# tanderson92/Fast_solver_Lippmann_Schwinger

Measured on NVIDIA B200. Metric: ls_operator_applies_per_s_2d, higher is better.
Workload: dtype f64

## Files before the change

fast_solver_lippmann_schwinger_b200/csrc/line_kernels.cuh:

```cuda
#pragma once
#include "fft_engine.cuh"
#include <cooperative_groups.h>

namespace lsk {
using namespace lsfft;

template <int N> struct GeoA {
    static constexpr int E = Cfg<N>::E;
    static constexpr int T = N / E;
    static constexpr int LPC = (T >= 128) ? 1 : 128 / T;
    static constexpr int THREADS = T * LPC;
};
template <int N> struct GeoB {
    static constexpr int E = Cfg<N>::E;
    static constexpr int T = N / E;
    static constexpr int LB = LinesB<N>::value;
    static constexpr int GPC = (LB * T >= 128) ? 1 : 128 / (LB * T);
    static constexpr int LPC = LB * GPC;
    static constexpr int THREADS = LB * T * GPC;
};
#ifndef LS_INV512_MINB
#define LS_INV512_MINB 2
#endif
template <int N, bool MODE_B> struct MinB {
    static constexpr int TH = MODE_B ? GeoB<N>::THREADS : GeoA<N>::THREADS;
    static constexpr int value = (TH <= 128) ? 3 : ((MODE_B && GeoB<N>::LB == 4 && TH == 256) ? 2 : 1);
};
template <int N, bool MODE_B> struct MinBInv {
    static constexpr int value = (N == 512 && MinB<N, MODE_B>::value == 3) ? LS_INV512_MINB : MinB<N, MODE_B>::value;
};

template <int N, bool MODE_B> struct Map;
template <int N> struct Map<N, false> {
    typedef GeoA<N> G;
    typedef LayA<N> Lay;
    int line, t;
    Lay lay;
    __device__ __forceinline__ Map() {
        line = threadIdx.x / G::T;
        t = threadIdx.x % G::T;
        lay.base = line * N;
    }
    __device__ __forceinline__ int lay_lam() const { return 0; }
};
template <int N> struct Map<N, true> {
    typedef GeoB<N> G;
    typedef LayB<N> Lay;
    int line, t;
    Lay lay;
    __device__ __forceinline__ Map() {
        constexpr int LB = G::LB;
        int grp = threadIdx.x / (LB * G::T);
        int w = threadIdx.x % (LB * G::T);
        lay.lam = w % LB;
        t = w / LB;
// ... 161 lines not shown
            cd gv[E];
            fft_fwd<N>(v, t, r, ex, mp.lay, tw, [&]() {
                const cd* g = MODE_B ? gsrc + ((long)(mp.line / LBK) * nr + rr) * UNIT + mp.lay_lam()
                                     : gsrc + ((long)mp.line * nr + rr) * UNIT;
                constexpr int gs = LBK;
#pragma unroll
                for (int e = 0; e < E; ++e) gv[e] = __ldg(&g[(t + T * e) * gs]);
            });
#pragma unroll
            for (int e = 0; e < E; ++e) v[e] = cmul(v[e], gv[e]);
        } else {
        fft_fwd<N>(v, t, r, ex, mp.lay, tw);
        mbar_wait(bar, (unsigned)(rr & 1));
        if (MODE_B) {
            const cd* g = gb + sm_group_off(mp);
#pragma unroll
            for (int e = 0; e < E; ++e) v[e] = cmul(v[e], g[(t + T * e) * LBK + mp.lay_lam()]);
        } else {
            const cd* g = gb + goff;
#pragma unroll
            for (int e = 0; e < E; ++e) v[e] = cmul(v[e], g[t + T * e]);
        }
        }
        fft_inv<N>(v, t, r, ex, mp.lay, tw, [&]() {
            if (GSM && rr + 1 < nr && threadIdx.x == 0) {
                fence_proxy_async();
                issue_g(rr + 1);
            }
        });
        if (ASM == 0) {
            demod_accumulate<N>(acc, v, r);
        } else if (r == 0) {
#pragma unroll
            for (int a = 0; a < AR; ++a) acc[a] = v[a];
#pragma unroll
            for (int a = AR; a < E; ++a) accs[(a - AR) * TH] = v[a];
        } else {
            acc[0] = cadd(acc[0], v[0]);
#pragma unroll
            for (int a = 1; a < AR; ++a) acc[a] = cfmac(v[a], c64(r * a * (16 / E)), acc[a]);
#pragma unroll
            for (int a = AR; a < E; ++a) accs[(a - AR) * TH] = cfmac(v[a], c64(r * a * (16 / E)), accs[(a - AR) * TH]);
        }
    }
    cd* o = out + line_out(la, L) + (long)t * la.out_es;
#pragma unroll
    for (int a = 0; a < AR; ++a) o[(long)(a * T) * la.out_es] = acc[a];
#pragma unroll
    for (int a = AR; a < E; ++a) o[(long)(a * T) * la.out_es] = accs[(a - AR) * TH];
}

template <int N, int MINB, int GL>
__global__ void __launch_bounds__(GeoA<N>::THREADS, MINB)
k_mid_swap(const cd* in, cd* out, const cd* __restrict__ G, const cd* __restrict__ TAB, const LineAddr la, long line0) {
    typedef Map<N, false> M;
    constexpr int E = Cfg<N>::E, T = N / E, LPC = M::G::LPC, TH = GeoA<N>::THREADS;
    extern __shared__ __align__(128) cd sm[];
    M mp;
    cd* ex = sm;
    cd* hold = sm + LPC * N + threadIdx.x;
    cd* tw1 = sm + 2 * LPC * N;
    load_tw1<N>(tw1, TAB);
    const long L = line0 + (long)blockIdx.x * LPC + mp.line;
    const int t = mp.t;
    const TwState<N> tw = make_tw<N>(t, TAB, tw1);
    const cd* gline = G + L * 2L * N;
    cd v[E];
    {
        const cd* p = in + line_in(la, L) + (long)t * la.in_es;
#pragma unroll
        for (int a = 0; a < E; ++a) v[a] = p[(long)(a * T) * la.in_es];
#pragma unroll
        for (int a = 0; a < E; ++a) hold[a * TH] = v[a];
    }
    __syncthreads();
#pragma unroll 1
    for (int rr = 0; rr < 2; ++rr) {
        const int r = 2 * rr;
        const cd* g = gline + (long)rr * N;
        if constexpr (GL == 0) {
            cd gv[E];
            fft_fwd<N>(v, t, r, ex, mp.lay, tw, [&]() {
#pragma unroll
                for (int e = 0; e < E; ++e) gv[e] = __ldg(&g[t + T * e]);
            });
#pragma unroll
            for (int e = 0; e < E; ++e) v[e] = cmul(v[e], gv[e]);
        } else {
            fft_fwd<N>(v, t, r, ex, mp.lay, tw, [&]() {
                if ((t & 7) == 0) {
#pragma unroll
                    for (int e = 0; e < E; ++e) prefetch_l2(&g[t + T * e]);
                }
            });
#pragma unroll
            for (int e = 0; e < E; ++e) v[e] = cmul(v[e], __ldg(&g[t + T * e]));
        }
        fft_inv<N>(v, t, r, ex, mp.lay, tw);
        if (rr == 0) {
#pragma unroll
            for (int a = 0; a < E; ++a) {
                const cd xa = hold[a * TH];
                hold[a * TH] = v[a];
                v[a] = xa;
            }
        }
    }
    cd* o = out + line_out(la, L) + (long)t * la.out_es;
    o[0] = cadd(hold[0], v[0]);
#pragma unroll
    for (int a = 1; a < E; ++a) o[(long)(a * T) * la.out_es] = cfmac(v[a], c64(2 * a * (16 / E)), hold[a * TH]);
}

__device__ __forceinline__ void cp_async16(void* dst_smem, const void* src) {
    asm volatile("cp.async.cg.shared.global [%0], [%1], 16;" ::"r"(smem_u32(dst_smem)), "l"(src) : "memory");
}
__device__ __forceinline__ void cp_async_commit() { asm volatile("cp.async.commit_group;" ::: "memory"); }
template <int K> __device__ __forceinline__ void cp_async_wait() { asm volatile("cp.async.wait_group %0;" ::"n"(K) : "memory"); }

template <int N, bool MODE_B, int PF = 0>
__global__ void __launch_bounds__(MODE_B ? GeoB<N>::THREADS : GeoA<N>::THREADS, MinBInv<N, MODE_B>::value)
k_inv_pruned(const cd* __restrict__ in, const cd* bsrc, cd* out, const cd* __restrict__ TAB, double scale,
             const LineAddr la, long line0) {
    typedef Map<N, MODE_B> M;
    constexpr int E = Cfg<N>::E, T = N / E, LPC = M::G::LPC;
    extern __shared__ __align__(128) cd sm[];
    M mp;
    cd* ex = sm + sm_group_off(mp);
    cd* tw1 = sm + LPC * N;
    load_tw1<N>(tw1, TAB);
    const long L = line0 + (long)blockIdx.x * LPC + mp.line;
    const int t = mp.t;
    const TwState<N> tw = make_tw<N>(t, TAB, tw1);
    __syncthreads();
    const long in_base = line_in(la, L), out_base = line_out(la, L);
    cd acc[E];
    const int nr = la.nr, rstep = 4 / la.nr;
    constexpr int TH = MODE_B ? GeoB<N>::THREADS : GeoA<N>::THREADS;
    cd* stg = sm + LPC * N + EngTab<N>::TW1N + threadIdx.x;
#pragma unroll 1
    for (int rr = 0; rr < nr; ++rr) {
        const int r = rr * rstep;
        cd v[E];
        const cd* p = in + in_base;
        if (PF == 2 && rr > 0) {
            cp_async_wait<0>();
#pragma unroll
            for (int e = 0; e < E; ++e) v[e] = stg[TH * e];
        } else {
#pragma unroll
            for (int e = 0; e < E; ++e) v[e] = p[slot_off(la, (long)(rr * N + t + T * e), la.in_es)];
        }
        if (PF == 2) {
            if (rr + 1 < nr) {
#pragma unroll
                for (int e = 0; e < E; ++e) cp_async16(&stg[TH * e], &p[slot_off(la, (long)((rr + 1) * N + t + T * e), la.in_es)]);
                cp_async_commit();
            } else if (bsrc != nullptr) {
#pragma unroll
                for (int a = 0; a < E; ++a) cp_async16(&stg[TH * a], &bsrc[out_base + (long)(a * T + t) * la.out_es]);
                cp_async_commit();
            }
        } else if (!PF) {
        } else if (rr + 1 < nr) {
// ... 12 lines not shown
    }
#pragma unroll
    for (int a = 0; a < E; ++a) {
        long off = out_base + (long)(a * T + t) * la.out_es;
        cd res = cscale(acc[a], scale);
        if (bsrc != nullptr) {
            if (PF == 2 && a == 0) cp_async_wait<0>();
            const cd bv = (PF == 2) ? stg[TH * a] : bsrc[off];
            res = make_double2(__fma_rn(acc[a].x, scale, bv.x), __fma_rn(acc[a].y, scale, bv.y));
        }
        out[off] = res;
    }
}

}

namespace lsk {

template <class K> inline cudaError_t smem_optin(K kernel, int smem, unsigned long long& done) {
    int dev = 0;
    cudaError_t e = cudaGetDevice(&dev);
    if (e != cudaSuccess) return e;
    const unsigned long long bit = 1ull << (dev & 63);
    if (done & bit) return cudaSuccess;
    e = cudaFuncSetAttribute(kernel, cudaFuncAttributeMaxDynamicSharedMemorySize, smem);
    if (e == cudaSuccess) done |= bit;
    return e;
}

template <int N, bool B>
inline cudaError_t launch_fwd(cudaStream_t s, long nlines, const cd* in, const double* nu, cd* out, const cd* TAB,
                              const LineAddr& la) {
    constexpr int smem = Smem<N, B>::fwd_bytes;
    constexpr int LPC = Smem<N, B>::LPC, TH = B ? GeoB<N>::THREADS : GeoA<N>::THREADS;
    static unsigned long long optin = 0;
    { cudaError_t e = smem_optin(k_fwd_pruned<N, B>, smem, optin); if (e != cudaSuccess) return e; }
    k_fwd_pruned<N, B><<<(unsigned)(nlines / LPC), TH, smem, s>>>(in, nu, out, TAB, la, 0);
    return cudaPeekAtLastError();
}

template <int N, bool B, bool GSM>
inline cudaError_t launch_mid(cudaStream_t s, long nlines, const cd* in, cd* out, const cd* G, const cd* TAB,
                              const LineAddr& la) {
    constexpr int smem = GSM ? Smem<N, B>::mid_bytes : Smem<N, B>::mid_bytes_direct;
    constexpr int LPC = Smem<N, B>::LPC, TH = B ? GeoB<N>::THREADS : GeoA<N>::THREADS;
    static unsigned long long optin = 0;
    constexpr int MB = (B && GeoB<N>::LB == 4) ? 2 : 1;
    { cudaError_t e = smem_optin(k_mid_fused<N, B, GSM, MB>, smem, optin); if (e != cudaSuccess) return e; }
    k_mid_fused<N, B, GSM, MB><<<(unsigned)(nlines / LPC), TH, smem, s>>>(in, out, G, TAB, la, 0);
    return cudaPeekAtLastError();
}

template <int N, int MINB, int GL>
inline cudaError_t launch_mid_swap(cudaStream_t s, long nlines, const cd* in, cd* out, const cd* G, const cd* TAB,
                                   const LineAddr& la) {
    constexpr int smem = (2 * GeoA<N>::LPC * N + EngTab<N>::TW1N) * (int)sizeof(cd);
    static unsigned long long optin = 0;
    { cudaError_t e = smem_optin(k_mid_swap<N, MINB, GL>, smem, optin); if (e != cudaSuccess) return e; }
    k_mid_swap<N, MINB, GL><<<(unsigned)(nlines / GeoA<N>::LPC), GeoA<N>::THREADS, smem, s>>>(in, out, G, TAB, la, 0);
    return cudaPeekAtLastError();
}

template <int N, bool B, int PF = 0>
inline cudaError_t launch_inv(cudaStream_t s, long nlines, const cd* in, const cd* bsrc, cd* out, const cd* TAB,
                              double scale, const LineAddr& la) {
    constexpr int smem = Smem<N, B>::fwd_bytes + (PF == 2 ? Smem<N, B>::LPC * N * (int)sizeof(cd) : 0);
    constexpr int LPC = Smem<N, B>::LPC, TH = B ? GeoB<N>::THREADS : GeoA<N>::THREADS;
    static unsigned long long optin = 0;
    { cudaError_t e = smem_optin(k_inv_pruned<N, B, PF>, smem, optin); if (e != cudaSuccess) return e; }
    k_inv_pruned<N, B, PF><<<(unsigned)(nlines / LPC), TH, smem, s>>>(in, bsrc, out, TAB, scale, la, 0);
    return cudaPeekAtLastError();
}

}
```

fast_solver_lippmann_schwinger_b200/csrc/op2d.cu:

```cuda
#include "ls_common.cuh"
#include "op2d_base.cuh"
#include "line_kernels.cuh"
#include "gv_spectrum2d.cuh"
#ifdef LS_EXPERIMENTS
#include "line_kernels_experiments.cuh"
#endif

using namespace ls;
using namespace lsk;

namespace {

struct Op2D : Op2DBase {
    int nr = 4;
    long pn = 0, pm = 0;
    double* d_nu = nullptr;
    cd* d_G = nullptr;
    cd* d_TABn = nullptr; cd* d_TABm = nullptr;
    cd* d_A = nullptr;
    cd* d_C = nullptr;
    int cw = 1;
    int apply_dev(const cd* b, cd* y, int mode) override;
};

__global__ void k_scale(cd* a, long n, double s) {
    for (long i = (long)blockIdx.x * blockDim.x + threadIdx.x; i < n; i += (long)gridDim.x * blockDim.x) {
        cd v = a[i];
        a[i] = make_double2(v.x * s, v.y * s);
    }
}

__global__ void k_permute_g2d(const cd* __restrict__ gin, cd* __restrict__ gout,
                              const int* __restrict__ fx, const int* __restrict__ fy,
                              long n, long m, long ne, long me, double scale) {
    long idx = (long)blockIdx.x * blockDim.x + threadIdx.x;
    long total = ne * me;
    if (idx >= total) return;
    long sy = idx % m;
    long ry = (idx / m) % 4;
    long sx = idx / (4 * m);
    long kx = 4L * fx[sx % n] + sx / n;
    long ky = 4L * fy[sy] + ry;
    long ix = (kx + ne / 2) % ne, iy = (ky + me / 2) % me;
    cd v = gin[ix + ne * iy];
    gout[idx] = make_double2(v.x * scale, v.y * scale);
}

__global__ void k_fill_g2d(cd* __restrict__ gout, const int* __restrict__ fx, const int* __restrict__ fy,
                           long n, long m, long ne, long me, double scale, Gv2dParams p) {
    long idx = (long)blockIdx.x * blockDim.x + threadIdx.x;
    long total = ne * me;
    if (idx >= total) return;
    long sy = idx % m;
    long ry = (idx / m) % 4;
    long sx = idx / (4 * m);
    long kx = 4L * fx[sx % n] + sx / n;
    long ky = 4L * fy[sy] + ry;
    long ix = (kx + ne / 2) % ne, iy = (ky + me / 2) % me;
    cd v = gtrunc2d_eval(p, ix, iy, ne, me);
    gout[idx] = make_double2(v.x * scale, v.y * scale);
}
__global__ void k_fill_g2d_centred(cd* __restrict__ gout, long ne, long me, Gv2dParams p) {
    long idx = (long)blockIdx.x * blockDim.x + threadIdx.x;
    if (idx >= ne * me) return;
    gout[idx] = gtrunc2d_eval(p, idx % ne, idx / ne, ne, me);
}

template <int N> int launch_fwd(Op2D* op, const cd* b, const double* nu) {
    constexpr int smem = Smem<N, false>::fwd_bytes;
    static unsigned long long optin = 0;
    LS_CUDA_TRY(smem_optin(k_fwd_pruned<N, false>, smem, optin));
    dim3 grid((unsigned)(op->m / GeoA<N>::LPC));
    LineAddr la{1L << 40, op->n, 0, 1, op->pn, 0, 1};
    la.nr = op->nr;
    op->phase_begin(0);
    k_fwd_pruned<N, false><<<grid, GeoA<N>::THREADS, smem, op->stream>>>(b, nu, op->d_A, op->d_TABn, la, 0);
    op->phase_end();
    op->launches++;
    return LS_OK;
}
template <int N, bool GSM, int MINB, int ASM = 0> int launch_mid_v(Op2D* op) {
    static int extra = -1;
    if (extra < 0) { const char* e = getenv("LS_P2_EXTRA_SMEM"); extra = e ? atoi(e) : 0; }
    const int smem = (GSM ? Smem<N, false>::mid_bytes : Smem<N, false>::mid_bytes_direct) + extra
                     + ASM * GeoA<N>::THREADS * (int)sizeof(cd);
    static unsigned long long optin = 0;
    LS_CUDA_TRY(smem_optin(k_mid_fused<N, false, GSM, MINB, ASM>, smem, optin));
    dim3 grid((unsigned)(op->pn / GeoA<N>::LPC));
    const long cw = op->cw;
    LineAddr la{cw, 1, cw, op->pn, 1, cw * op->m, cw};
    la.nr = op->nr;
    op->phase_begin(1);
    k_mid_fused<N, false, GSM, MINB, ASM><<<grid, GeoA<N>::THREADS, smem, op->stream>>>(
        op->d_A, op->d_C, op->d_G, op->d_TABm, la, 0);
    op->phase_end();
    op->launches++;
    return LS_OK;
}
#ifdef LS_EXPERIMENTS
template <int N, int ASM> int launch_mid_dual(Op2D* op) {
    const int smem = (3 * GeoA<N>::LPC * N + EngTab<N>::TW1N + ASM * GeoA<N>::THREADS) * (int)sizeof(cd);
    static unsigned long long optin = 0;
    LS_CUDA_TRY(smem_optin(k_mid_fused_dual<N, ASM>, smem, optin));
    dim3 grid((unsigned)(op->ne / GeoA<N>::LPC));
    op->phase_begin(1);
    k_mid_fused_dual<N, ASM><<<grid, GeoA<N>::THREADS, smem, op->stream>>>(
        op->d_A, op->d_C, op->d_G, op->d_TABm, LineAddr{1L << 40, 1, 0, op->ne, op->m, 0, 1}, 0);
    op->phase_end();
    op->launches++;
    return LS_OK;
}
#endif
template <int N> int launch_mid_swap_op(Op2D* op) {
    const long cw = op->cw;
    LineAddr la{cw, 1, cw, op->pn, 1, cw * op->m, cw};
    la.nr = 2;
    static int gl = -1, minb = -1;
    if (gl < 0) { const char* e = getenv("LS_P2_GLOAD"); gl = e ? atoi(e) : 0; }
    if (minb < 0) { const char* e = getenv("LS_P2_MINB"); minb = e ? atoi(e) : 0; }
    const int use_minb = minb ? minb : (N <= 256 ? 3 : 2);
    constexpr int MB = (GeoA<N>::THREADS <= 128 ? 3 : 1);
    op->phase_begin(1);
    cudaError_t e;
    constexpr int MB2 = (MB == 3 ? 2 : 1);
    if (use_minb == 2 || MB == 1) e = gl ? lsk::launch_mid_swap<N, MB2, 1>(op->stream, op->pn, op->d_A, op->d_C, op->d_G, op->d_TABm, la)
                                     : lsk::launch_mid_swap<N, MB2, 0>(op->stream, op->pn, op->d_A, op->d_C, op->d_G, op->d_TABm, la);
    else e = gl ? lsk::launch_mid_swap<N, MB, 1>(op->stream, op->pn, op->d_A, op->d_C, op->d_G, op->d_TABm, la)
                : lsk::launch_mid_swap<N, MB, 0>(op->stream, op->pn, op->d_A, op->d_C, op->d_G, op->d_TABm, la);
    op->phase_end();
    op->launches++;
    LS_CUDA_TRY(e);
    return LS_OK;
}
template <int N> int launch_mid(Op2D* op) {
    static int kernel = -1;
    if (kernel < 0) { const char* e = getenv("LS_P2_KERNEL"); kernel = e ? atoi(e) : 1; }
    if (op->nr == 2 && kernel == 1) return launch_mid_swap_op<N>(op);
#ifndef LS_EXPERIMENTS
    return launch_mid_v<N, false, 1>(op);
#else
    static int variant = -1;
    if (op->nr != 4) return launch_mid_v<N, false, 1>(op);
    if (variant < 0) { const char* e = getenv("LS_P2_VARIANT"); variant = e ? atoi(e) : 1; }
    if (variant == 0) return launch_mid_v<N, true, 1>(op);
    if constexpr (N == 2048) if (variant == 8) {
        static int ctas = -1;
        if (ctas < 0) { const char* e = getenv("LS_P2_CTAS"); ctas = e ? atoi(e) : 2 * 148; }
        op->phase_begin(1);
        cudaError_t e = launch_mid_persist<N>(op->stream, op->ne, op->d_A, op->d_C, op->d_G, op->d_TABm,
                                              LineAddr{1L << 40, 1, 0, op->ne, op->m, 0, 1}, ctas);
        op->phase_end();
        op->launches++;
        LS_CUDA_TRY(e);
        return LS_OK;
    }
    if constexpr (N == 2048) if (variant == 6 || variant == 7) {
        op->phase_begin(1);
        const LineAddr la{1L << 40, 1, 0, op->ne, op->m, 0, 1};
        cudaError_t e = (variant == 6) ? launch_mid_cluster<N, false, 3>(op->stream, op->ne, op->d_A, op->d_C, op->d_G, op->d_TABm, la)
                                       : launch_mid_cluster<N, false, 4>(op->stream, op->ne, op->d_A, op->d_C, op->d_G, op->d_TABm, la);
        op->phase_end();
        op->launches++;
        LS_CUDA_TRY(e);
        return LS_OK;
    }
    if constexpr (N == 2048) { if (variant == 5) return launch_mid_dual<N, 4>(op); }
    if (variant == 2) return launch_mid_v<N, false, 3, 4>(op);
    if (variant == 3) return launch_mid_v<N, false, 3, 2>(op);
    return launch_mid_v<N, false, 1>(op);
#endif
}
template <int N, int PF> int launch_inv_v(Op2D* op, const cd* bsrc, cd* y, double scale) {
    constexpr int smem = Smem<N, false>::fwd_bytes + (PF == 2 ? Smem<N, false>::LPC * N * (int)sizeof(cd) : 0);
    static unsigned long long optin = 0;
    LS_CUDA_TRY(smem_optin(k_inv_pruned<N, false, PF>, smem, optin));
    dim3 grid((unsigned)(op->m / GeoA<N>::LPC));
    const long cw = op->cw;
    int cshift = 0;
    while ((1L << cshift) < cw) ++cshift;
    LineAddr la{1L << 40, cw, 0, 1, op->n, 0, 1};
    la.split_shift = cshift; la.split_stride = cw * op->m;
    la.nr = op->nr;
    op->phase_begin(2);
    k_inv_pruned<N, false, PF><<<grid, GeoA<N>::THREADS, smem, op->stream>>>(op->d_C, bsrc, y, op->d_TABn, scale, la, 0);
    op->phase_end();
    op->launches++;
    return LS_OK;
}
template <int N> int launch_inv(Op2D* op, const cd* bsrc, cd* y, double scale) {
    static int stage = -1;
// ... 50 lines not shown
    }

int compact_spectrum(Op2D* op, cd* g4s) {
    const long n = op->n, m = op->m;
    cudaStream_t s = op->stream;
    cudaError_t e = cudaSuccess;
    cd *t1 = nullptr, *g2 = nullptr, *t2 = nullptr, *G2 = nullptr;
    int rc;
    if ((rc = op->dmalloc((void**)&t1, (size_t)(4 * n) * (2 * m) * sizeof(cd)))) return rc;
    for (int c = 0; c <= 3; c += 3) {
        LineAddr la{1L << 40, 4 * m, 0, 1, 2 * m, 0, 1};
        la.nr = 4; la.cblock = c;
        cd* outp = t1 + (c ? m : 0);
#define S1(N) launch_inv<N, false>(s, 4 * n, g4s, nullptr, outp, op->d_TABm, 1.0, la)
        LS_DISPATCH_E(m, S1);
        LS_CUDA_TRY(e);
    }
    LS_CUDA_TRY(cudaStreamSynchronize(s));
    op->dfree(g4s);
    if ((rc = op->dmalloc((void**)&g2, (size_t)(2 * n) * (2 * m) * sizeof(cd)))) return rc;
    for (int c = 0; c <= 3; c += 3) {
        LineAddr la{1L << 40, 1, 0, 2 * m, 2 * n, 0, 1};
        la.nr = 4; la.cblock = c;
        cd* outp = g2 + (c ? n : 0);
#define S2(N) launch_inv<N, false>(s, 2 * m, t1, nullptr, outp, op->d_TABn, 1.0, la)
        LS_DISPATCH_E(n, S2);
        LS_CUDA_TRY(e);
    }
    LS_CUDA_TRY(cudaStreamSynchronize(s));
    op->dfree(t1);
    if ((rc = op->dmalloc((void**)&t2, (size_t)(2 * n) * (2 * m) * sizeof(cd)))) return rc;
    if ((rc = op->dmalloc((void**)&G2, (size_t)(2 * n) * (2 * m) * sizeof(cd)))) return rc;
    {
        LineAddr la{1L << 40, 2 * n, 0, 1, 2 * n, 0, 1};
        la.nr = 2; la.full2 = 1;
#define S3(N) launch_fwd<N, false>(s, 2 * m, g2, nullptr, t2, op->d_TABn, la)
        LS_DISPATCH_E(n, S3);
        LS_CUDA_TRY(e);
    }
    {
        LineAddr la{1L << 40, 1, 0, 2 * n, 2 * m, 0, 1};
        la.nr = 2; la.full2 = 1;
#define S4(N) launch_fwd<N, false>(s, 2 * n, t2, nullptr, G2, op->d_TABm, la)
        LS_DISPATCH_E(m, S4);
        LS_CUDA_TRY(e);
    }
    k_scale<<<148 * 8, 256, 0, s>>>(G2, (2 * n) * (2 * m), 1.0 / ((double)(2 * n) * (double)(2 * m)));
    LS_CUDA_TRY(cudaStreamSynchronize(s));
    op->dfree(g2);
    op->dfree(t2);
    op->d_G = G2;
    op->nr = 2;
    return LS_OK;
}

}

extern "C" {

static int op2d_create_impl(ls_handle* out, int64_t n, int64_t m, int64_t ne, int64_t me,
                            const double* nu, const ls_cdouble* gfft, double omega, int quadrule, int flags,
                            double L, double Lp);

int ls_op2d_create(ls_handle* out, int64_t n, int64_t m, int64_t ne, int64_t me,
                   const double* nu, const ls_cdouble* gfft, double omega, int quadrule, int flags) {
    LS_REQUIRE(out && nu && gfft, LS_ERR_INVALID, "ls_op2d_create: null pointer");
    return op2d_create_impl(out, n, m, ne, me, nu, gfft, omega, quadrule, flags, 0.0, 0.0);
}

int ls_op2d_create_gv(ls_handle* out, int64_t n, int64_t m, const double* nu, double omega, double L, double Lp, int flags) {
    LS_REQUIRE(out && nu, LS_ERR_INVALID, "ls_op2d_create_gv: null pointer");
    LS_REQUIRE(L > 0 && Lp > 0 && omega > 0, LS_ERR_INVALID, "ls_op2d_create_gv: L, Lp and k must be positive");
    return op2d_create_impl(out, n, m, 4 * n, 4 * m, nu, nullptr, omega, LS_QUAD_GREENGARD_VICO, flags, L, Lp);
}

static int op2d_create_impl(ls_handle* out, int64_t n, int64_t m, int64_t ne, int64_t me,
                            const double* nu, const ls_cdouble* gfft, double omega, int quadrule, int flags,
                            double L, double Lp) {
    LS_REQUIRE(n > 0 && m > 0 && ne > 0 && me > 0, LS_ERR_INVALID, "ls_op2d_create: non-positive size");
    LS_REQUIRE(quadrule == LS_QUAD_TRAPEZOIDAL || quadrule == LS_QUAD_GREENGARD_VICO, LS_ERR_INVALID,
               "ls_op2d_create: unknown quadRule %d", quadrule);
    if (quadrule == LS_QUAD_TRAPEZOIDAL) {
        LS_REQUIRE(ne == 2 * n - 1 && me == 2 * m - 1, LS_ERR_INVALID,
                   "ls_op2d_create: trapezoidal needs ne = 2n-1, me = 2m-1 (FastConvolution.jl:183)");
        return create_op2d_generic(out, n, m, ne, me, nu, gfft, omega, quadrule);
    }
    LS_REQUIRE(ne == 4 * n && me == 4 * m, LS_ERR_INVALID,
               "ls_op2d_create: Greengard_Vico needs ne = 4n, me = 4m (FastConvolution.jl:201)");
    if (!(fft_size_supported(n) && fft_size_supported(m)) || (flags & LS_FLAG_FORCE_GENERIC)) {
        if (gfft) return create_op2d_generic(out, n, m, ne, me, nu, gfft, omega, quadrule);
        LS_REQUIRE(ne + n - 1 <= 4096 && me + m - 1 <= 4096, LS_ERR_UNSUPPORTED,
                   "ls_op2d_create_gv: n=%ld, m=%ld: the general-size GPU path serves 5n - 1 <= 4096", (long)n, (long)m);
        cd* d_g = nullptr;
        LS_CUDA_TRY(cudaMalloc((void**)&d_g, (size_t)ne * me * sizeof(cd)));
        const Gv2dParams gp = gv2d_params(L, Lp, omega);
        k_fill_g2d_centred<<<(unsigned)(((size_t)ne * me + 255) / 256), 256>>>(d_g, ne, me, gp);
        cudaError_t ge = cudaDeviceSynchronize();
        int grc = ge == cudaSuccess ? create_op2d_generic(out, n, m, ne, me, nu, nullptr, omega, quadrule, d_g) : LS_ERR_CUDA;
        if (ge != cudaSuccess) set_error("spectrum generation failed: %s", cudaGetErrorString(ge));
        cudaFree(d_g);
        return grc;
    }

    Op2D* op = new Op2D();
    int rc = op->init_base(KIND_OP2D);
    if (rc) { delete op; return rc; }
    op->n = n; op->m = m; op->ne = ne; op->me = me; op->omega = omega; op->quadrule = quadrule;
    const size_t N = (size_t)n * m, NE = (size_t)ne * me;
#define TRY(x) do { rc = (x); if (rc) { delete op; return rc; } } while (0)
    TRY(op->dupload((void**)&op->d_nu, nu, N * sizeof(double)));
    {
        auto Tn = engine_table((int)n), Tm = engine_table((int)m);
        TRY(op->dupload((void**)&op->d_TABn, Tn.data(), Tn.size() * sizeof(cd)));
        TRY(op->dupload((void**)&op->d_TABm, Tm.data(), Tm.size() * sizeof(cd)));
    }
    {
        auto fx = slot_freq((int)n), fy = slot_freq((int)m);
        int *d_fx = nullptr, *d_fy = nullptr;
        cd* d_gin = nullptr;
        TRY(op->dupload((void**)&d_fx, fx.data(), fx.size() * sizeof(int)));
        TRY(op->dupload((void**)&d_fy, fy.data(), fy.size() * sizeof(int)));
        TRY(op->dmalloc((void**)&op->d_G, NE * sizeof(cd)));
        const int th = 256;
        if (gfft) {
            TRY(op->dupload((void**)&d_gin, gfft, NE * sizeof(cd)));
            k_permute_g2d<<<(unsigned)((NE + th - 1) / th), th, 0, op->stream>>>(
                d_gin, op->d_G, d_fx, d_fy, n, m, ne, me, 1.0 / ((double)ne * (double)me));
        } else {
            k_fill_g2d<<<(unsigned)((NE + th - 1) / th), th, 0, op->stream>>>(
                op->d_G, d_fx, d_fy, n, m, ne, me, 1.0 / ((double)ne * (double)me), gv2d_params(L, Lp, omega));
        }
        cudaError_t e = cudaStreamSynchronize(op->stream);
        if (e != cudaSuccess) { set_error("spectrum set-up failed: %s", cudaGetErrorString(e)); delete op; return LS_ERR_CUDA; }
        if (d_gin) op->dfree(d_gin);
        op->dfree(d_fx); op->dfree(d_fy);
    }
    op->nr = 4;
    if (!(flags & LS_FLAG_PAD4)) {
        cd* g4s = op->d_G;
        op->d_G = nullptr;
        TRY(compact_spectrum(op, g4s));
    }
    op->pn = op->nr * n; op->pm = op->nr * m;
    {
        const char* ev = getenv("LS_C_INTERLEAVE");
        int cw = ev ? atoi(ev) : 4;
        if (cw != 1 && cw != 2 && cw != 4 && cw != 8) cw = 4;
        const char* pv = getenv("LS_P2_VARIANT");
        if (op->nr == 4 && pv && atoi(pv) >= 5) cw = 1;
        op->cw = cw;
    }
    TRY(op->dmalloc((void**)&op->d_A, (size_t)op->pn * m * sizeof(cd)));
    TRY(op->dmalloc((void**)&op->d_C, (size_t)op->pn * m * sizeof(cd)));
    TRY(op->dmalloc((void**)&op->d_b, N * sizeof(cd)));
    TRY(op->dmalloc((void**)&op->d_y, N * sizeof(cd)));
#undef TRY
    *out = reinterpret_cast<ls_handle>(op);
    return LS_OK;
}

int ls_op2d_apply(ls_handle h, const ls_cdouble* b, ls_cdouble* y, int mode, int memloc) {
    LS_REQUIRE(h && b && y, LS_ERR_INVALID, "ls_op2d_apply: null argument");
    Op2DBase* op = reinterpret_cast<Op2DBase*>(h);
    LS_REQUIRE(op->kind == KIND_OP2D, LS_ERR_INVALID, "ls_op2d_apply: not a 2-D operator handle");
    LS_REQUIRE(mode == LS_APPLY_FASTCONVOLUTION || mode == LS_APPLY_FFTCONVOLUTION, LS_ERR_INVALID,
               "ls_op2d_apply: unknown mode %d", mode);
    if (mode == LS_APPLY_FFTCONVOLUTION)
        LS_REQUIRE(op->n == op->m, LS_ERR_INVALID,
                   "FFTconvolution pads (ne,ne) and crops (n,n): square grids only (FastConvolution.jl:139-151)");
    LS_CUDA_TRY(cudaSetDevice(op->device));
    const size_t bytes = (size_t)op->n * op->m * sizeof(cd);
    if (memloc == LS_MEM_DEVICE) {
        return op->apply_dev(reinterpret_cast<const cd*>(b), reinterpret_cast<cd*>(y), mode);
    }
    LS_REQUIRE(memloc == LS_MEM_HOST, LS_ERR_INVALID, "ls_op2d_apply: unknown memloc %d", memloc);
    LS_CUDA_TRY(cudaMemcpyAsync(op->d_b, b, bytes, cudaMemcpyHostToDevice, op->stream));
    int rc = op->apply_dev(op->d_b, op->d_y, mode);
    if (rc) return rc;
    LS_CUDA_TRY(cudaMemcpyAsync(y, op->d_y, bytes, cudaMemcpyDeviceToHost, op->stream));
    LS_CUDA_TRY(cudaStreamSynchronize(op->stream));
    return LS_OK;
}

}
```

fast_solver_lippmann_schwinger_b200/_lib.py:

```python
from __future__ import annotations

import ctypes as C
import os
import re

import numpy as np

HERE = os.path.dirname(os.path.abspath(__file__))
LIB_PATH = os.environ.get("LS_CUDA_LIB") or os.path.join(HERE, "lib", "libls_cuda.so")
HEADER_PATH = os.path.join(os.path.dirname(HERE), "include", "ls_cuda.h")

LS_OK = 0
LS_ERR_INVALID, LS_ERR_UNSUPPORTED, LS_ERR_CUDA, LS_ERR_NOMEM, LS_ERR_NCCL, LS_ERR_CALLBACK = -1, -2, -3, -4, -5, -6
MEM_HOST, MEM_DEVICE = 0, 1
QUAD_TRAPEZOIDAL, QUAD_GREENGARD_VICO = 0, 1
APPLY_FASTCONVOLUTION, APPLY_FFTCONVOLUTION = 0, 1

QUADRULES = {"trapezoidal": QUAD_TRAPEZOIDAL, "Greengard_Vico": QUAD_GREENGARD_VICO}


class CDouble(C.Structure):
    _fields_ = [("re", C.c_double), ("im", C.c_double)]

    @classmethod
# ... 37 lines not shown
    vp, i64, dbl, ci = C.c_void_p, C.c_int64, C.c_double, C.c_int
    sig = {
        "ls_version": (ci, []),
        "ls_last_error": (C.c_char_p, []),
        "ls_device_count": (ci, [C.POINTER(ci)]),
        "ls_set_device": (ci, [ci]),
        "ls_dev_alloc": (ci, [C.POINTER(vp), C.c_size_t]),
        "ls_dev_free": (ci, [vp]),
        "ls_memcpy_h2d": (ci, [vp, vp, C.c_size_t]),
        "ls_memcpy_d2h": (ci, [vp, vp, C.c_size_t]),
        "ls_host_alloc_pinned": (ci, [C.POINTER(vp), C.c_size_t]),
        "ls_host_free_pinned": (ci, [vp]),
        "ls_op2d_create": (ci, [C.POINTER(vp), i64, i64, i64, i64, vp, vp, dbl, ci, ci]),
        "ls_op2d_create_gv": (ci, [C.POINTER(vp), i64, i64, vp, dbl, dbl, dbl, ci]),
        "ls_op2d_apply": (ci, [vp, vp, vp, ci, ci]),
        "ls_op3d_create": (ci, [C.POINTER(vp), i64, i64, i64, i64, i64, i64, vp, vp, dbl, dbl, dbl, ci]),
        "ls_op3d_apply": (ci, [vp, vp, vp, ci, ci]),
        "ls_op3d_info": (ci, [vp, C.POINTER(ci), C.POINTER(ci), C.POINTER(ci)]),
        "ls_nccl_unique_id": (ci, [vp]),
        "ls_op3d_create_dist": (ci, [C.POINTER(vp), i64, i64, i64, vp, dbl, dbl, dbl, ci, ci, vp, ci]),
        "ls_op_size": (ci, [vp, C.POINTER(i64)]),
        "ls_spm_create": (ci, [C.POINTER(vp), i64, i64, vp, vp, vp]),
        "ls_spm_create_dist": (ci, [C.POINTER(vp), vp, i64, i64, vp, vp, vp]),
        "ls_spm_mv": (ci, [vp, CDouble, vp, CDouble, vp, ci]),
        "ls_spm_info": (ci, [vp, C.POINTER(i64), C.POINTER(i64), C.POINTER(i64), C.POINTER(ci), C.POINTER(ci)]),
        "ls_krylov_create": (ci, [C.POINTER(vp), i64]),
        "ls_krylov_set_orth": (ci, [vp, ci]),
        "ls_zdotc": (ci, [vp, vp, vp, C.POINTER(CDouble)]),
        "ls_dznrm2": (ci, [vp, vp, C.POINTER(dbl)]),
        "ls_zaxpy": (ci, [vp, CDouble, vp, vp]),
        "ls_zscal": (ci, [vp, CDouble, vp]),
        "ls_mgs_step": (ci, [vp, vp, i64, ci, vp, vp]),
        "ls_gmres": (ci, [vp, vp, vp, SOLVE_CB, vp, vp, vp, ci, i64, dbl, dbl, ci, vp, i64,
                          C.POINTER(i64), C.POINTER(ci), C.POINTER(i64), ci]),
        "ls_msp_factor": (ci, [C.POINTER(vp), i64, i64, vp, vp, vp]),
        "ls_msp_factor3d": (ci, [C.POINTER(vp), i64, i64, i64, vp, vp, vp]),
        "ls_msp_solve": (ci, [vp, vp, vp, ci]),
        "ls_msp_info": (ci, [vp, C.POINTER(i64), C.POINTER(ci), C.POINTER(dbl)]),
        "ls_msp_plan": (ci, [vp, C.c_char_p, i64]),
        "ls_gmres_msp": (ci, [vp, vp, vp, vp, vp, vp, ci, i64, dbl, dbl, ci, vp, i64,
                              C.POINTER(i64), C.POINTER(ci), C.POINTER(i64), ci]),
        "ls_krylov_last_precond_host_seconds": (ci, [vp, C.POINTER(dbl)]),
        "ls_sample_rows": (ci, [vp, vp, vp, ci, vp, i64]),
        "ls_gram": (ci, [vp, vp, i64, ci, vp]),
        "ls_gather_rows": (ci, [vp, vp, i64, ci, vp, ci, vp]),
        "ls_destroy": (ci, [vp]),
        "ls_sync": (ci, [vp]),
        "ls_timer_start": (ci, [vp]),
        "ls_timer_stop": (ci, [vp, C.POINTER(C.c_float)]),
        "ls_launch_count": (ci, [vp, C.POINTER(i64)]),
        "ls_profile_enable": (ci, [vp, ci]),
        "ls_profile_read": (ci, [vp, C.POINTER(dbl), C.POINTER(i64), ci]),
        "ls_test_fft_lines": (ci, [i64, i64, vp, vp, ci]),
        "ls_test_device_peaks": (ci, [C.POINTER(dbl), C.POINTER(dbl), C.POINTER(dbl)]),
    }
    for name, (res, args) in sig.items():
        fn = getattr(L, name)
        fn.restype = res
        fn.argtypes = args
    L._signatures = sig
    _lib = L
    return L


def check(rc):
    if rc == LS_OK:
        return
    msg = lib().ls_last_error().decode("utf-8", "replace")
    if rc == LS_ERR_UNSUPPORTED:
        raise LSUnsupported(rc, msg)
    raise LSCudaError(rc, msg)


def ptr(a):
    if a is None:
        return None
    if isinstance(a, np.ndarray):
        return a.ctypes.data_as(C.c_void_p)
    if isinstance(a, DeviceBuffer):
        return C.c_void_p(a.ptr)
    return C.c_void_p(int(a))


class DeviceBuffer:

    def __init__(self, nbytes):
        p = C.c_void_p()
        check(lib().ls_dev_alloc(C.byref(p), nbytes))
        self.ptr = p.value
        self.nbytes = nbytes

    @classmethod
    def from_host(cls, arr):
        arr = np.ascontiguousarray(arr)
        buf = cls(arr.nbytes)
        check(lib().ls_memcpy_h2d(C.c_void_p(buf.ptr), ptr(arr), arr.nbytes))
        return buf

    def to_host(self, dtype=np.complex128, count=None):
        dtype = np.dtype(dtype)
        count = self.nbytes // dtype.itemsize if count is None else count
        out = np.empty(count, dtype=dtype)
        check(lib().ls_memcpy_d2h(ptr(out), C.c_void_p(self.ptr), count * dtype.itemsize))
        return out

    def offset(self, nbytes):
# ... 37 lines not shown
```

include/ls_cuda.h:

```cpp
#ifndef LS_CUDA_H
#define LS_CUDA_H

#include <stddef.h>
#include <stdint.h>

#ifdef __cplusplus
extern "C" {
#endif

typedef struct { double re, im; } ls_cdouble;
typedef struct ls_handle_s* ls_handle;

#define LS_OK               0
#define LS_ERR_INVALID     -1
#define LS_ERR_UNSUPPORTED -2
#define LS_ERR_CUDA        -3
#define LS_ERR_NOMEM       -4
#define LS_ERR_NCCL        -5
#define LS_ERR_CALLBACK    -6

#define LS_FLAG_FORCE_GENERIC 1
#define LS_FLAG_PAD4          2

#define LS_MEM_HOST   0
// ... 35 lines not shown
int ls_op3d_apply(ls_handle h, const ls_cdouble* b, ls_cdouble* y, int mode, int memloc);

int ls_spm_create(ls_handle* out, int64_t nrows, int64_t ncols, const int64_t* colptr,
                  const int64_t* rowval, const ls_cdouble* nzval);
int ls_spm_create_dist(ls_handle* out, ls_handle op, int64_t nrows_local, int64_t halo, const int64_t* colptr,
                       const int64_t* rowval, const ls_cdouble* nzval);
int ls_spm_mv(ls_handle A, ls_cdouble alpha, const ls_cdouble* x, ls_cdouble beta, ls_cdouble* y, int memloc);
int ls_spm_info(ls_handle A, int64_t* nrows, int64_t* ncols, int64_t* nnz, int* format, int* nclasses);

int ls_krylov_create(ls_handle* out, int64_t n);
int ls_krylov_set_orth(ls_handle k, int orth_meth);
int ls_zdotc(ls_handle k, const ls_cdouble* x, const ls_cdouble* y, ls_cdouble* result);
int ls_dznrm2(ls_handle k, const ls_cdouble* x, double* result);
int ls_zaxpy(ls_handle k, ls_cdouble alpha, const ls_cdouble* x, ls_cdouble* y);
int ls_zscal(ls_handle k, ls_cdouble alpha, ls_cdouble* x);
int ls_mgs_step(ls_handle k, const ls_cdouble* V, int64_t ldv, int kcols, ls_cdouble* w, ls_cdouble* hcol);

typedef int (*ls_solve_cb)(void* user, ls_cdouble* v_inout, int64_t n);

int ls_gmres(ls_handle krylov, ls_handle op, ls_handle As, ls_solve_cb msp_solve, void* user,
             const ls_cdouble* b, ls_cdouble* x, int restart, int64_t maxiter, double reltol,
             double abstol, int initially_zero, double* resnorm_hist, int64_t hist_cap,
             int64_t* niter, int* converged, int64_t* mv_products, int memloc);

int ls_msp_factor(ls_handle* out, int64_t n, int64_t m, const int64_t* colptr, const int64_t* rowval,
                  const ls_cdouble* nzval);
int ls_msp_factor3d(ls_handle* out, int64_t n, int64_t m, int64_t l, const int64_t* colptr, const int64_t* rowval,
                    const ls_cdouble* nzval);
int ls_msp_solve(ls_handle msp, const ls_cdouble* rhs, ls_cdouble* x, int memloc);
int ls_msp_info(ls_handle msp, int64_t* factor_bytes, int* depth, double* factor_seconds);
int ls_msp_plan(ls_handle msp, char* buf, int64_t cap);
int ls_gmres_msp(ls_handle krylov, ls_handle op, ls_handle As, ls_handle msp,
                 const ls_cdouble* b, ls_cdouble* x, int restart, int64_t maxiter, double reltol,
                 double abstol, int initially_zero, double* resnorm_hist, int64_t hist_cap,
                 int64_t* niter, int* converged, int64_t* mv_products, int memloc);
int ls_krylov_last_precond_host_seconds(ls_handle krylov, double* seconds);

int ls_sample_rows(ls_handle krylov, ls_handle op, const int64_t* indS, int s, ls_cdouble* V_dev, int64_t ldv);
int ls_gram(ls_handle krylov, const ls_cdouble* V_dev, int64_t ldv, int s, ls_cdouble* gram_host);
int ls_gather_rows(ls_handle krylov, const ls_cdouble* V_dev, int64_t ldv, int s, const int64_t* idx, int nidx, ls_cdouble* out_host);

int ls_destroy(ls_handle h);
int ls_sync(ls_handle h);
int ls_timer_start(ls_handle h);
int ls_timer_stop(ls_handle h, float* elapsed_ms);
int ls_launch_count(ls_handle h, int64_t* count);

int ls_profile_enable(ls_handle h, int on);
int ls_profile_read(ls_handle h, double* ms_per_phase, int64_t* launches_per_phase, int nphase);

int ls_test_fft_lines(int64_t N, int64_t nlines, const ls_cdouble* in_host, ls_cdouble* out_host,
                      int inverse_roundtrip);

int ls_test_device_peaks(double* dfma_tflops, double* dadd_tinst, double* copy_gbs);

#ifdef __cplusplus
}
#endif
#endif
```

Before: 2846.

## Add TMA-tiled mid-phase kernel loading transposed line tiles via tensor maps

Adds a new middle-stage kernel that uses TMA bulk tensor loads to pull a tile of strided lines into swizzled shared memory. It then runs the forward FFT, spectrum multiply and inverse FFT in place and writes the tile back with TMA 3D stores into the interleaved C layout. The goal is to replace scattered strided global accesses with coalesced bulk copies and cut address-generation overhead. It becomes the default for sizes 1024–2048 when tensor maps encode successfully. In exchange it adds shared memory for the tile and serialises the load, compute and store phases within each CTA.

Result: faster. 2960 (median of 6 runs) (+4.0%).

```diff
diff --git a/fast_solver_lippmann_schwinger_b200/csrc/line_kernels.cuh b/fast_solver_lippmann_schwinger_b200/csrc/line_kernels.cuh
--- a/fast_solver_lippmann_schwinger_b200/csrc/line_kernels.cuh
+++ b/fast_solver_lippmann_schwinger_b200/csrc/line_kernels.cuh
@@ -1,6 +1,7 @@
 #pragma once
 #include "fft_engine.cuh"
 #include <cooperative_groups.h>
+#include <cuda.h>
 
 namespace lsk {
 using namespace lsfft;
@@ -326,6 +327,101 @@
     o[0] = cadd(hold[0], v[0]);
 #pragma unroll
     for (int a = 1; a < E; ++a) o[(long)(a * T) * la.out_es] = cfmac(v[a], c64(2 * a * (16 / E)), hold[a * TH]);
+}
+
+template <int N> struct TileA {
+    static constexpr int LPC = GeoA<N>::LPC;
+    static constexpr int LT = LPC > 2 ? LPC : 2;
+    static constexpr int ROWS = N < 256 ? N : 256;
+    static constexpr int TW1N = EngTab<N>::TW1N;
+    static constexpr int smem_bytes = ((LT + LPC) * N + TW1N) * (int)sizeof(cd) + 16;
+};
+__device__ __forceinline__ int tile_swz(int k, int cwt) { return k ^ ((k >> 3) & (cwt - 1)); }
+
+__device__ __forceinline__ void tma_load_2d(void* dst_smem, const CUtensorMap* map, int x, int y, unsigned long long* bar) {
+    asm volatile("cp.async.bulk.tensor.2d.shared::cluster.global.tile.mbarrier::complete_tx::bytes [%0], [%1, {%2, %3}], [%4];"
+                 ::"r"(smem_u32(dst_smem)), "l"(map), "r"(x), "r"(y), "r"(smem_u32(bar)) : "memory");
+}
+__device__ __forceinline__ void tma_store_3d(const CUtensorMap* map, int x, int y, int z, const void* src_smem) {
+    asm volatile("cp.async.bulk.tensor.3d.global.shared::cta.bulk_group [%0, {%1, %2, %3}], [%4];"
+                 ::"l"(map), "r"(x), "r"(y), "r"(z), "r"(smem_u32(src_smem)) : "memory");
+}
+
+template <int N, int MINB>
+__global__ void __launch_bounds__(GeoA<N>::THREADS, MINB)
+k_mid_tile(const __grid_constant__ CUtensorMap tmA, const __grid_constant__ CUtensorMap tmC, const cd* __restrict__ G,
+           const cd* __restrict__ TAB, int cwl, int cwtl) {
+    typedef Map<N, false> M;
+    typedef TileA<N> TG;
+    constexpr int E = Cfg<N>::E, T = N / E, LPC = TG::LPC, LT = TG::LT, ROWS = TG::ROWS;
+    extern __shared__ __align__(1024) cd smt[];
+    cd* tile = smt;
+    cd* ex = smt + LT * N;
+    cd* tw1 = ex + LPC * N;
+    unsigned long long* bar = reinterpret_cast<unsigned long long*>(tw1 + TG::TW1N);
+    const int cwt = 1 << cwtl;
+    const int sx0 = blockIdx.x * LT;
+    if (threadIdx.x == 0) {
+        mbar_init(bar, 1);
+        mbar_expect_tx(bar, (unsigned)(LT * N * sizeof(cd)));
+        for (int g = 0; g < LT >> cwtl; ++g)
+            for (int j0 = 0; j0 < N; j0 += ROWS)
+                tma_load_2d(tile + ((g * N + j0) << cwtl), &tmA, 2 * (sx0 + (g << cwtl)), j0, bar);
+    }
+    M mp;
+    load_tw1<N>(tw1, TAB);
+    const int t = mp.t;
+    const TwState<N> tw = make_tw<N>(t, TAB, tw1);
+    __syncthreads();
+    mbar_wait(bar, 0);
+#pragma unroll 1
+    for (int q = mp.line; q < LT; q += LPC) {
+        const int k0 = ((q >> cwtl) * N << cwtl) + (q & (cwt - 1));
+        const cd* gline = G + (long)(sx0 + q) * 2L * N;
+        cd v[E];
+#pragma unroll
+        for (int a = 0; a < E; ++a) v[a] = tile[tile_swz(k0 + ((a * T + t) << cwtl), cwt)];
+#pragma unroll 1
+        for (int rr = 0; rr < 2; ++rr) {
+            const int r = 2 * rr;
+            const cd* g = gline + (long)rr * N;
+            cd gv[E];
+            fft_fwd<N>(v, t, r, ex, mp.lay, tw, [&]() {
+#pragma unroll
+                for (int e = 0; e < E; ++e) gv[e] = __ldg(&g[t + T * e]);
+            });
+#pragma unroll
+            for (int e = 0; e < E; ++e) v[e] = cmul(v[e], gv[e]);
+            fft_inv<N>(v, t, r, ex, mp.lay, tw);
+            if (rr == 0) {
+#pragma unroll
+                for (int a = 0; a < E; ++a) {
+                    cd* h = &tile[tile_swz(k0 + ((a * T + t) << cwtl), cwt)];
+                    const cd xa = *h;
+                    *h = v[a];
+                    v[a] = xa;
+                }
+            }
+        }
+        tile[tile_swz(k0 + (t << cwtl), cwt)] = cadd(tile[tile_swz(k0 + (t << cwtl), cwt)], v[0]);
+#pragma unroll
+        for (int a = 1; a < E; ++a) {
+            cd* h = &tile[tile_swz(k0 + ((a * T + t) << cwtl), cwt)];
+            *h = cfmac(v[a], c64(2 * a * (16 / E)), *h);
+        }
+    }
+    fence_proxy_async();
+    __syncthreads();
+    if (threadIdx.x == 0) {
+        const int cw = 1 << cwl;
+        for (int g = 0; g < LT >> cwtl; ++g) {
+            const int sx = sx0 + (g << cwtl);
+            for (int j0 = 0; j0 < N; j0 += ROWS)
+                tma_store_3d(&tmC, 2 * (sx & (cw - 1)), j0, sx >> cwl, tile + ((g * N + j0) << cwtl));
+        }
+        asm volatile("cp.async.bulk.commit_group;" ::: "memory");
+        asm volatile("cp.async.bulk.wait_group.read 0;" ::: "memory");
+    }
 }
 
 __device__ __forceinline__ void cp_async16(void* dst_smem, const void* src) {
@@ -453,6 +549,16 @@
     return cudaPeekAtLastError();
 }
 
+template <int N, int MINB>
+inline cudaError_t launch_mid_tile(cudaStream_t s, long nlines, const CUtensorMap& tmA, const CUtensorMap& tmC, const cd* G,
+                                   const cd* TAB, int cwl, int cwtl) {
+    constexpr int smem = TileA<N>::smem_bytes;
+    static unsigned long long optin = 0;
+    { cudaError_t e = smem_optin(k_mid_tile<N, MINB>, smem, optin); if (e != cudaSuccess) return e; }
+    k_mid_tile<N, MINB><<<(unsigned)(nlines / TileA<N>::LT), GeoA<N>::THREADS, smem, s>>>(tmA, tmC, G, TAB, cwl, cwtl);
+    return cudaPeekAtLastError();
+}
+
 template <int N, bool B, int PF = 0>
 inline cudaError_t launch_inv(cudaStream_t s, long nlines, const cd* in, const cd* bsrc, cd* out, const cd* TAB,
                               double scale, const LineAddr& la) {
diff --git a/fast_solver_lippmann_schwinger_b200/csrc/op2d.cu b/fast_solver_lippmann_schwinger_b200/csrc/op2d.cu
--- a/fast_solver_lippmann_schwinger_b200/csrc/op2d.cu
+++ b/fast_solver_lippmann_schwinger_b200/csrc/op2d.cu
@@ -2,6 +2,7 @@
 #include "op2d_base.cuh"
 #include "line_kernels.cuh"
 #include "gv_spectrum2d.cuh"
+#include <cudaTypedefs.h>
 #ifdef LS_EXPERIMENTS
 #include "line_kernels_experiments.cuh"
 #endif
@@ -20,6 +21,9 @@
     cd* d_A = nullptr;
     cd* d_C = nullptr;
     int cw = 1;
+    CUtensorMap tmA, tmC;
+    bool tiles = false;
+    int cwl = 0, cwtl = 0;
     int apply_dev(const cd* b, cd* y, int mode) override;
 };
 
@@ -132,10 +136,21 @@
     LS_CUDA_TRY(e);
     return LS_OK;
 }
+template <int N> int launch_mid_tile_op(Op2D* op) {
+    constexpr int MB = N <= 256 ? 3 : (GeoA<N>::THREADS <= 128 ? 2 : 1);
+    op->phase_begin(1);
+    cudaError_t e = lsk::launch_mid_tile<N, MB>(op->stream, op->pn, op->tmA, op->tmC, op->d_G, op->d_TABm, op->cwl, op->cwtl);
+    op->phase_end();
+    op->launches++;
+    LS_CUDA_TRY(e);
+    return LS_OK;
+}
 template <int N> int launch_mid(Op2D* op) {
     static int kernel = -1;
-    if (kernel < 0) { const char* e = getenv("LS_P2_KERNEL"); kernel = e ? atoi(e) : 1; }
-    if (op->nr == 2 && kernel == 1) return launch_mid_swap_op<N>(op);
+    if (kernel < 0) { const char* e = getenv("LS_P2_KERNEL"); kernel = e ? atoi(e) : 3; }
+    if constexpr (N <= 2048)
+        if (op->nr == 2 && op->tiles && (kernel == 2 || (kernel == 3 && N >= 1024))) return launch_mid_tile_op<N>(op);
+    if (op->nr == 2 && kernel >= 1) return launch_mid_swap_op<N>(op);
 #ifndef LS_EXPERIMENTS
     return launch_mid_v<N, false, 1>(op);
 #else
@@ -292,6 +307,36 @@
     op->d_G = G2;
     op->nr = 2;
     return LS_OK;
+}
+
+template <int N> int encode_tile_maps(Op2D* op) {
+    static PFN_cuTensorMapEncodeTiled_v12000 encode = nullptr;
+    if (!encode) {
+        void* fn = nullptr;
+        cudaDriverEntryPointQueryResult q;
+        if (cudaGetDriverEntryPointByVersion("cuTensorMapEncodeTiled", &fn, 12000, cudaEnableDefault, &q) != cudaSuccess
+            || q != cudaDriverEntryPointSuccess || !fn)
+            return 0;
+        encode = reinterpret_cast<PFN_cuTensorMapEncodeTiled_v12000>(fn);
+    }
+    const int cw = op->cw, cwt = TileA<N>::LT < cw ? TileA<N>::LT : cw;
+    op->cwl = 0; while ((1 << op->cwl) < cw) ++op->cwl;
+    op->cwtl = 0; while ((1 << op->cwtl) < cwt) ++op->cwtl;
+    const CUtensorMapSwizzle swz = cwt == 1 ? CU_TENSOR_MAP_SWIZZLE_NONE
+                                 : cwt == 2 ? CU_TENSOR_MAP_SWIZZLE_32B : cwt == 4 ? CU_TENSOR_MAP_SWIZZLE_64B : CU_TENSOR_MAP_SWIZZLE_128B;
+    const cuuint64_t pn = op->pn, m = op->m, es = sizeof(cd);
+    const cuuint32_t rows = TileA<N>::ROWS, ones[3] = {1, 1, 1};
+    const cuuint64_t dA[2] = {2 * pn, m}, sA[1] = {pn * es};
+    const cuuint32_t bA[2] = {(cuuint32_t)(2 * cwt), rows};
+    const cuuint64_t dC[3] = {2 * (cuuint64_t)cw, m, pn / cw}, sC[2] = {cw * es, cw * m * es};
+    const cuuint32_t bC[3] = {(cuuint32_t)(2 * cwt), rows, 1};
+    if (encode(&op->tmA, CU_TENSOR_MAP_DATA_TYPE_FLOAT64, 2, op->d_A, dA, sA, bA, ones, CU_TENSOR_MAP_INTERLEAVE_NONE, swz,
+               CU_TENSOR_MAP_L2_PROMOTION_NONE, CU_TENSOR_MAP_FLOAT_OOB_FILL_NONE) != CUDA_SUCCESS)
+        return 0;
+    if (encode(&op->tmC, CU_TENSOR_MAP_DATA_TYPE_FLOAT64, 3, op->d_C, dC, sC, bC, ones, CU_TENSOR_MAP_INTERLEAVE_NONE, swz,
+               CU_TENSOR_MAP_L2_PROMOTION_NONE, CU_TENSOR_MAP_FLOAT_OOB_FILL_NONE) != CUDA_SUCCESS)
+        return 0;
+    return 1;
 }
 
 }
@@ -392,6 +437,13 @@
     }
     TRY(op->dmalloc((void**)&op->d_A, (size_t)op->pn * m * sizeof(cd)));
     TRY(op->dmalloc((void**)&op->d_C, (size_t)op->pn * m * sizeof(cd)));
+    if (op->nr == 2) {
+#define ENC(N_) encode_tile_maps<N_>(op)
+        LS_DISPATCH_N(op->m, ENC);
+#undef ENC
+        op->tiles = rc == 1;
+        rc = LS_OK;
+    }
     TRY(op->dmalloc((void**)&op->d_b, N * sizeof(cd)));
     TRY(op->dmalloc((void**)&op->d_y, N * sizeof(cd)));
 #undef TRY
```

## Exploit mirror symmetry of Green's spectrum and pair mirrored lines per block

Applied to the files above, without the earlier changes.

At setup, a device kernel checks whether the compacted Green's function spectrum is symmetric under frequency mirroring. If it is, the mid-stage kernel reads mirrored rows through an index table so both lines of a pair use the same G row. Lines are also reordered so each block processes a line and its mirror together, aiming to improve L2 reuse of G and cut its memory traffic. The cost is an extra indirection load per line and a gathered access pattern on the input lines.

After: 2806 before, 2801 after, median of 6. No clear change (-0.2%).

```diff
diff --git a/fast_solver_lippmann_schwinger_b200/_lib.py b/fast_solver_lippmann_schwinger_b200/_lib.py
--- a/fast_solver_lippmann_schwinger_b200/_lib.py
+++ b/fast_solver_lippmann_schwinger_b200/_lib.py
@@ -113,6 +113,7 @@
         "ls_profile_enable": (ci, [vp, ci]),
         "ls_profile_read": (ci, [vp, C.POINTER(dbl), C.POINTER(i64), ci]),
         "ls_test_fft_lines": (ci, [i64, i64, vp, vp, ci]),
+        "ls_test_op2d_spectrum_rows": (ci, [vp, C.POINTER(i64)]),
         "ls_test_device_peaks": (ci, [C.POINTER(dbl), C.POINTER(dbl), C.POINTER(dbl)]),
     }
     for name, (res, args) in sig.items():
diff --git a/fast_solver_lippmann_schwinger_b200/csrc/line_kernels.cuh b/fast_solver_lippmann_schwinger_b200/csrc/line_kernels.cuh
--- a/fast_solver_lippmann_schwinger_b200/csrc/line_kernels.cuh
+++ b/fast_solver_lippmann_schwinger_b200/csrc/line_kernels.cuh
@@ -268,7 +268,8 @@
 
 template <int N, int MINB, int GL>
 __global__ void __launch_bounds__(GeoA<N>::THREADS, MINB)
-k_mid_swap(const cd* in, cd* out, const cd* __restrict__ G, const cd* __restrict__ TAB, const LineAddr la, long line0) {
+k_mid_swap(const cd* in, cd* out, const cd* __restrict__ G, const int* __restrict__ lorder, const int* __restrict__ grow,
+           const cd* __restrict__ TAB, const LineAddr la) {
     typedef Map<N, false> M;
     constexpr int E = Cfg<N>::E, T = N / E, LPC = M::G::LPC, TH = GeoA<N>::THREADS;
     extern __shared__ __align__(128) cd sm[];
@@ -277,10 +278,10 @@
     cd* hold = sm + LPC * N + threadIdx.x;
     cd* tw1 = sm + 2 * LPC * N;
     load_tw1<N>(tw1, TAB);
-    const long L = line0 + (long)blockIdx.x * LPC + mp.line;
+    const long L = __ldg(&lorder[(long)blockIdx.x * LPC + mp.line]);
     const int t = mp.t;
     const TwState<N> tw = make_tw<N>(t, TAB, tw1);
-    const cd* gline = G + L * 2L * N;
+    const cd* gline = G + (long)__ldg(&grow[L]) * 2L * N;
     cd v[E];
     {
         const cd* p = in + line_in(la, L) + (long)t * la.in_es;
@@ -444,12 +445,12 @@
 }
 
 template <int N, int MINB, int GL>
-inline cudaError_t launch_mid_swap(cudaStream_t s, long nlines, const cd* in, cd* out, const cd* G, const cd* TAB,
-                                   const LineAddr& la) {
+inline cudaError_t launch_mid_swap(cudaStream_t s, long nlines, const cd* in, cd* out, const cd* G, const int* lorder,
+                                   const int* grow, const cd* TAB, const LineAddr& la) {
     constexpr int smem = (2 * GeoA<N>::LPC * N + EngTab<N>::TW1N) * (int)sizeof(cd);
     static unsigned long long optin = 0;
     { cudaError_t e = smem_optin(k_mid_swap<N, MINB, GL>, smem, optin); if (e != cudaSuccess) return e; }
-    k_mid_swap<N, MINB, GL><<<(unsigned)(nlines / GeoA<N>::LPC), GeoA<N>::THREADS, smem, s>>>(in, out, G, TAB, la, 0);
+    k_mid_swap<N, MINB, GL><<<(unsigned)(nlines / GeoA<N>::LPC), GeoA<N>::THREADS, smem, s>>>(in, out, G, lorder, grow, TAB, la);
     return cudaPeekAtLastError();
 }
 
diff --git a/fast_solver_lippmann_schwinger_b200/csrc/op2d.cu b/fast_solver_lippmann_schwinger_b200/csrc/op2d.cu
--- a/fast_solver_lippmann_schwinger_b200/csrc/op2d.cu
+++ b/fast_solver_lippmann_schwinger_b200/csrc/op2d.cu
@@ -1,3 +1,5 @@
+#include <algorithm>
+#include <cstring>
 #include "ls_common.cuh"
 #include "op2d_base.cuh"
 #include "line_kernels.cuh"
@@ -16,6 +18,9 @@
     long pn = 0, pm = 0;
     double* d_nu = nullptr;
     cd* d_G = nullptr;
+    int* d_lorder = nullptr;
+    int* d_grow = nullptr;
+    long g_rows = 0;
     cd* d_TABn = nullptr; cd* d_TABm = nullptr;
     cd* d_A = nullptr;
     cd* d_C = nullptr;
@@ -123,10 +128,10 @@
     op->phase_begin(1);
     cudaError_t e;
     constexpr int MB2 = (MB == 3 ? 2 : 1);
-    if (use_minb == 2 || MB == 1) e = gl ? lsk::launch_mid_swap<N, MB2, 1>(op->stream, op->pn, op->d_A, op->d_C, op->d_G, op->d_TABm, la)
-                                     : lsk::launch_mid_swap<N, MB2, 0>(op->stream, op->pn, op->d_A, op->d_C, op->d_G, op->d_TABm, la);
-    else e = gl ? lsk::launch_mid_swap<N, MB, 1>(op->stream, op->pn, op->d_A, op->d_C, op->d_G, op->d_TABm, la)
-                : lsk::launch_mid_swap<N, MB, 0>(op->stream, op->pn, op->d_A, op->d_C, op->d_G, op->d_TABm, la);
+    if (use_minb == 2 || MB == 1) e = gl ? lsk::launch_mid_swap<N, MB2, 1>(op->stream, op->pn, op->d_A, op->d_C, op->d_G, op->d_lorder, op->d_grow, op->d_TABm, la)
+                                     : lsk::launch_mid_swap<N, MB2, 0>(op->stream, op->pn, op->d_A, op->d_C, op->d_G, op->d_lorder, op->d_grow, op->d_TABm, la);
+    else e = gl ? lsk::launch_mid_swap<N, MB, 1>(op->stream, op->pn, op->d_A, op->d_C, op->d_G, op->d_lorder, op->d_grow, op->d_TABm, la)
+                : lsk::launch_mid_swap<N, MB, 0>(op->stream, op->pn, op->d_A, op->d_C, op->d_G, op->d_lorder, op->d_grow, op->d_TABm, la);
     op->phase_end();
     op->launches++;
     LS_CUDA_TRY(e);
@@ -294,6 +299,68 @@
     return LS_OK;
 }
 
+__global__ void k_mirror_dev(const cd* __restrict__ G, const int* __restrict__ mir, long rows, long len,
+                             unsigned long long* out) {
+    double dmax = 0.0, gmax = 0.0;
+    for (long i = (long)blockIdx.x * blockDim.x + threadIdx.x; i < rows * len; i += (long)gridDim.x * blockDim.x) {
+        const long r = i / len, k = i % len;
+        const cd a = G[i], b = G[(long)mir[r] * len + k];
+        dmax = fmax(dmax, hypot(a.x - b.x, a.y - b.y));
+        gmax = fmax(gmax, hypot(a.x, a.y));
+    }
+    for (int o = 16; o > 0; o >>= 1) {
+        dmax = fmax(dmax, __shfl_xor_sync(0xffffffffu, dmax, o));
+        gmax = fmax(gmax, __shfl_xor_sync(0xffffffffu, gmax, o));
+    }
+    if ((threadIdx.x & 31) == 0) {
+        atomicMax(&out[0], (unsigned long long)__double_as_longlong(dmax));
+        atomicMax(&out[1], (unsigned long long)__double_as_longlong(gmax));
+    }
+}
+
+int mirror_tables(Op2D* op) {
+    const long n = op->n, pn = 2 * n, len = 2 * op->m;
+    const auto fx = slot_freq((int)n);
+    std::vector<int> sinv(n), mir(pn), lorder, grow(pn);
+    for (long i = 0; i < n; ++i) sinv[fx[i]] = (int)i;
+    for (long sx = 0; sx < pn; ++sx) {
+        const long b = sx / n, f = fx[sx % n];
+        mir[sx] = (int)(b * n + sinv[b == 0 ? (n - f) % n : n - 1 - f]);
+    }
+    const int z0 = sinv[0], zh = sinv[n / 2];
+    std::vector<char> seen(pn, 0);
+    for (long sx = 0; sx < pn; ++sx) {
+        if (seen[sx]) continue;
+        const int p = (sx == z0) ? zh : (sx == zh ? z0 : mir[sx]);
+        lorder.push_back((int)sx);
+        lorder.push_back(p);
+        seen[sx] = seen[p] = 1;
+    }
+    int* d_mir = nullptr;
+    unsigned long long* d_out = nullptr;
+    int rc;
+    if ((rc = op->dupload((void**)&d_mir, mir.data(), mir.size() * sizeof(int)))) return rc;
+    if ((rc = op->dmalloc((void**)&d_out, 2 * sizeof(unsigned long long)))) return rc;
+    LS_CUDA_TRY(cudaMemsetAsync(d_out, 0, 2 * sizeof(unsigned long long), op->stream));
+    k_mirror_dev<<<148 * 8, 256, 0, op->stream>>>(op->d_G, d_mir, pn, len, d_out);
+    unsigned long long h[2];
+    LS_CUDA_TRY(cudaMemcpyAsync(h, d_out, sizeof(h), cudaMemcpyDeviceToHost, op->stream));
+    LS_CUDA_TRY(cudaStreamSynchronize(op->stream));
+    op->dfree(d_mir);
+    op->dfree(d_out);
+    double dmax, gmax;
+    memcpy(&dmax, &h[0], sizeof(double));
+    memcpy(&gmax, &h[1], sizeof(double));
+    op->g_rows = 0;
+    const bool sym = dmax <= 1e-12 * gmax;
+    for (long sx = 0; sx < pn; ++sx) {
+        grow[sx] = sym ? std::min<int>((int)sx, mir[sx]) : (int)sx;
+        op->g_rows += (grow[sx] == sx);
+    }
+    if ((rc = op->dupload((void**)&op->d_lorder, lorder.data(), lorder.size() * sizeof(int)))) return rc;
+    return op->dupload((void**)&op->d_grow, grow.data(), grow.size() * sizeof(int));
+}
+
 }
 
 extern "C" {
@@ -380,6 +447,7 @@
         cd* g4s = op->d_G;
         op->d_G = nullptr;
         TRY(compact_spectrum(op, g4s));
+        TRY(mirror_tables(op));
     }
     op->pn = op->nr * n; op->pm = op->nr * m;
     {
@@ -396,6 +464,15 @@
     TRY(op->dmalloc((void**)&op->d_y, N * sizeof(cd)));
 #undef TRY
     *out = reinterpret_cast<ls_handle>(op);
+    return LS_OK;
+}
+
+int ls_test_op2d_spectrum_rows(ls_handle h, int64_t* rows) {
+    LS_REQUIRE(h && rows, LS_ERR_INVALID, "ls_test_op2d_spectrum_rows: null argument");
+    Op2DBase* base = reinterpret_cast<Op2DBase*>(h);
+    LS_REQUIRE(base->kind == KIND_OP2D, LS_ERR_INVALID, "ls_test_op2d_spectrum_rows: not a 2-D operator handle");
+    Op2D* op = dynamic_cast<Op2D*>(base);
+    *rows = op ? op->g_rows : 0;
     return LS_OK;
 }
 
diff --git a/include/ls_cuda.h b/include/ls_cuda.h
--- a/include/ls_cuda.h
+++ b/include/ls_cuda.h
@@ -111,6 +111,8 @@
 int ls_test_fft_lines(int64_t N, int64_t nlines, const ls_cdouble* in_host, ls_cdouble* out_host,
                       int inverse_roundtrip);
 
+int ls_test_op2d_spectrum_rows(ls_handle h, int64_t* rows);
+
 int ls_test_device_peaks(double* dfma_tflops, double* dadd_tinst, double* copy_gbs);
 
 #ifdef __cplusplus
```
